# Takatsuka-Mark/Photogrammetry

Measured on AMD Instinct MI355X. Metric: descriptor pairs matched/sec, higher is better.
Workload: dtype u8 / bits (descriptor bits expanded to fp4 +-1 for the MFMA distance: exact integers in f32 accumulators; integer keys); f32 grey; 1 GPU; BASELINE configs[2] (SURVEY 8d config 3) x 1: 64-frame 1920x1080 RGBA64 sequence(s), dewarp(shipped coeffs)+gray+FAST(T=0.1)+NMS(r=16; SURVEY 8d writes r = 20 for this config: both leave more than 4096 survivors per frame, the lists are cut to the same length either way)+BRIEF-256 per frame, all 2016 ordered image pairs per sequence through the greedy Hamming match, <=4096 keypoints per frame (fir; frames=64, image_pairs=2016, frames_per_gpu=64, image_pairs_per_gpu=2016, parallelism=frames f mod 1, image pairs p mod 1; 2 all-gathers per step (elided at N = 1), jobs_in_flight=2, rehearsal_on_one_gpu_with_gloo=False

## Files before the change

### photogrammetry_amd/csrc/k_image.hip

```cpp
#include "pgx_internal.h"

namespace {

__device__ __forceinline__ float gray_of(uint2 px)
{
    float r = (float)(px.x & 0xFFFFu), g = (float)(px.x >> 16), b = (float)(px.y & 0xFFFFu);
    float s = __fadd_rn(__fadd_rn(r, b), g);
    return __fdiv_rn(s, 196605.0f);
}

constexpr int FB = 4;

__device__ __forceinline__ uint2 widen8(uint32_t v)
{
    return make_uint2(__builtin_amdgcn_perm(v, v, 0x01010000u), __builtin_amdgcn_perm(v, v, 0x03030202u));
}

template <bool SRC8> struct SrcPix { using type = uint2; };
template <> struct SrcPix<true> { using type = uint32_t; };
template <bool SRC8> __device__ __forceinline__ uint2 load_px(const typename SrcPix<SRC8>::type *p);
template <> __device__ __forceinline__ uint2 load_px<false>(const uint2 *p) { return *p; }
template <> __device__ __forceinline__ uint2 load_px<true>(const uint32_t *p) { return widen8(*p); }

template <bool HAS_MAP, bool WRITE_RGBA, bool SRC8>
__global__ __launch_bounds__(256) void k_dewarp_gray(const typename SrcPix<SRC8>::type *__restrict__ rgba,
                                                     const int2 *__restrict__ map, int W, int H, int F,
                                                     float *__restrict__ gray, uint2 *__restrict__ dewarped, int *status)
{
    using Px = typename SrcPix<SRC8>::type;
    const size_t npix = (size_t)W * H;
    const int f0 = blockIdx.y * FB;
    const int nf = F - f0 < FB ? F - f0 : FB;
    const size_t ngroups = (npix + 3) / 4;
    const bool vec = (npix & 3) == 0 || F == 1;
    bool oob = false;
    for (size_t grp = (size_t)blockIdx.x * blockDim.x + threadIdx.x; grp < ngroups;
         grp += (size_t)gridDim.x * blockDim.x) {
        const size_t i0 = grp * 4;
        if (vec && i0 + 3 < npix) {
            size_t so[4];
            bool ok[4];
            if (HAS_MAP) {
                const int4 m01 = *reinterpret_cast<const int4 *>(map + i0);
                const int4 m23 = *reinterpret_cast<const int4 *>(map + i0 + 2);
                const int us[4] = {m01.x, m01.z, m23.x, m23.z};
                const int vs[4] = {m01.y, m01.w, m23.y, m23.w};
#pragma unroll
                for (int k = 0; k < 4; k++) {
                    const unsigned su = (unsigned)us[k] & 0xFFFFu, sv = (unsigned)vs[k] & 0xFFFFu;
                    ok[k] = su < (unsigned)W && sv < (unsigned)H;
                    oob |= !ok[k];
                    so[k] = ok[k] ? (size_t)sv * W + su : 0;
                }
            }
            uint2 px[FB][4];
#pragma unroll
            for (int fb = 0; fb < FB; fb++) {
                if (fb >= nf) break;
                const Px *src = rgba + (size_t)(f0 + fb) * npix;
                if (HAS_MAP) {
#pragma unroll
                    for (int k = 0; k < 4; k++) px[fb][k] = load_px<SRC8>(src + so[k]);
                } else if constexpr (SRC8) {
                    const uint4 a = *reinterpret_cast<const uint4 *>(src + i0);
                    px[fb][0] = widen8(a.x); px[fb][1] = widen8(a.y); px[fb][2] = widen8(a.z); px[fb][3] = widen8(a.w);
                } else {
                    const uint4 a = *reinterpret_cast<const uint4 *>(src + i0);
                    const uint4 b = *reinterpret_cast<const uint4 *>(src + i0 + 2);
                    px[fb][0] = make_uint2(a.x, a.y); px[fb][1] = make_uint2(a.z, a.w);
                    px[fb][2] = make_uint2(b.x, b.y); px[fb][3] = make_uint2(b.z, b.w);
                }
            }
#pragma unroll
            for (int fb = 0; fb < FB; fb++) {
                if (fb >= nf) break;
                if (HAS_MAP) {
#pragma unroll
                    for (int k = 0; k < 4; k++) if (!ok[k]) px[fb][k] = make_uint2(0, 0);
                }
                if (gray) {
                    const float4 g4 = make_float4(gray_of(px[fb][0]), gray_of(px[fb][1]), gray_of(px[fb][2]), gray_of(px[fb][3]));
                    *reinterpret_cast<float4 *>(gray + (size_t)(f0 + fb) * npix + i0) = g4;
                }
                if (WRITE_RGBA) {
                    uint2 *dout = dewarped + (size_t)(f0 + fb) * npix;
                    *reinterpret_cast<uint4 *>(dout + i0) = make_uint4(px[fb][0].x, px[fb][0].y, px[fb][1].x, px[fb][1].y);
                    *reinterpret_cast<uint4 *>(dout + i0 + 2) = make_uint4(px[fb][2].x, px[fb][2].y, px[fb][3].x, px[fb][3].y);
                }
            }
        } else {
            for (size_t i = i0; i < npix && i < i0 + 4; i++) {
                size_t o = i;
                bool okk = true;
                if (HAS_MAP) {
                    const int2 m = map[i];
                    const unsigned su = (unsigned)m.x & 0xFFFFu, sv = (unsigned)m.y & 0xFFFFu;
                    okk = su < (unsigned)W && sv < (unsigned)H;
                    oob |= !okk;
                    o = okk ? (size_t)sv * W + su : 0;
                }
                for (int fb = 0; fb < nf; fb++) {
                    const uint2 p = okk ? load_px<SRC8>(rgba + (size_t)(f0 + fb) * npix + o) : make_uint2(0, 0);
                    if (gray) gray[(size_t)(f0 + fb) * npix + i] = gray_of(p);
                    if (WRITE_RGBA) dewarped[(size_t)(f0 + fb) * npix + i] = p;
                }
            }
        }
    }
    if (HAS_MAP && oob) atomicOr(status, (int)PGX_ST_OOB_SOURCE);
}

__device__ __forceinline__ int32_t trunc_to_int_dev(double v)
{
    if (!(v > -2147483649.0 && v < 2147483648.0)) return INT32_MIN;
    return (int32_t)v;
}

__device__ __forceinline__ double cbrt_signed_dev(double n)
{
    const double sgn = (double)((n > 0) - (n < 0));
    return pow(fabs(n), 1.0 / 3.0) * sgn;
}

__global__ __launch_bounds__(256) void k_dewarp_map(int W, int H, double k0, double k1, double k2, double k3, double k4,
                                                    int2 *__restrict__ map, int *status)
{
    const size_t i = (size_t)blockIdx.x * 256 + threadIdx.x;
    if (i >= (size_t)W * H) return;
    const int v = (int)(i / W), u = (int)(i - (size_t)v * W);
    const double x0 = W / 2.0, y0 = H / 2.0;
    const int x = trunc_to_int_dev(u - x0), y = trunc_to_int_dev(v - y0);
    const int rd2 = x * x + y * y;
    const double rd = sqrt((double)rd2);
    const double den = rd * k4 - k1;
    const double a2 = (rd * k3 - k0) / den, a1 = (rd * k2 - 1) / den, a0 = rd / den;
    const double Q = (3 * a1 - a2 * a2) / 9.0;
    const double R = (9.0 * a2 * a1 - 27 * a0 - 2 * a2 * a2 * a2) / 54.0;
    const double Q3 = Q * Q * Q;
    const double D = Q3 + R * R;
    const double shift = -a2 / 3.0;
    const double nan = __longlong_as_double(0x7FF8000000000000ll);
    double r0 = nan, r1 = nan, r2 = nan;
    if (D >= 0) {
        const double sqrtD = pow(D, 0.5);
        const double S = cbrt_signed_dev(R + sqrtD), T = cbrt_signed_dev(R - sqrtD);
        r0 = shift + (S + T);
        if (D == 0) r1 = shift - S;
    } else {
        const double pi = 3.1415926535897932384626433832795;
        const double theta = acos(R / sqrt(-Q3));
        const double m = 2.0 * sqrt(-Q);
        r0 = m * cos(theta / 3.0) + shift;
        r1 = m * cos((theta + 2.0 * pi) / 3.0) + shift;
        r2 = m * cos((theta - 2.0 * pi) / 3.0) + shift;
    }
    double kept[3];
    int n = 0;
    if (!isnan(r0)) kept[n++] = r0;
    if (!isnan(r1)) kept[n++] = r1;
    if (!isnan(r2)) kept[n++] = r2;
    if (n == 0) { atomicOr(status, (int)PGX_ST_INTERNAL); map[i] = make_int2(INT32_MIN, INT32_MIN); return; }
    if (n >= 2 && kept[0] > kept[1]) { const double t = kept[0]; kept[0] = kept[1]; kept[1] = t; }
    if (n == 3) {
        if (kept[1] > kept[2]) { const double t = kept[1]; kept[1] = kept[2]; kept[2] = t; }
        if (kept[0] > kept[1]) { const double t = kept[0]; kept[0] = kept[1]; kept[1] = t; }
    }
    const double root = n == 3 ? kept[1] : kept[0];
    const double theta = atan2((double)y, (double)x);
    map[i] = make_int2(trunc_to_int_dev(root * cos(theta) + x0), trunc_to_int_dev(root * sin(theta) + y0));
}

}

void pgx_launch_dewarp_gray(hipStream_t s, const void *rgba, int src8, const int32_t *map_uv, int F, int W, int H,
                            float *gray, uint16_t *dewarped, int *status)
{
    if (F <= 0 || W <= 0 || H <= 0) return;
    const size_t ngroups = ((size_t)W * H + 3) / 4;
    unsigned gx = (unsigned)((ngroups + 255) / 256);
    const unsigned ny = (unsigned)((F + FB - 1) / FB);
    const unsigned cap = 512u / ny > 32u ? 512u / ny : 32u;
    if (gx > cap) gx = cap;
    dim3 grid(gx, (unsigned)((F + FB - 1) / FB)), block(256);
    const int2 *map = reinterpret_cast<const int2 *>(map_uv);
    uint2 *dw = reinterpret_cast<uint2 *>(dewarped);
#define PGX_DG(M, WR, S8) hipLaunchKernelGGL((k_dewarp_gray<M, WR, S8>), grid, block, 0, s, \
                                             reinterpret_cast<const SrcPix<S8>::type *>(rgba), map, W, H, F, gray, dw, status)
    if (src8) {
        if (map) { if (dw) PGX_DG(true, true, true); else PGX_DG(true, false, true); }
        else { if (dw) PGX_DG(false, true, true); else PGX_DG(false, false, true); }
    } else {
        if (map) { if (dw) PGX_DG(true, true, false); else PGX_DG(true, false, false); }
        else { if (dw) PGX_DG(false, true, false); else PGX_DG(false, false, false); }
    }
#undef PGX_DG
}

void pgx_launch_dewarp_map(hipStream_t s, int W, int H, const double *k, int32_t *map_uv, int *status)
{
    const size_t npix = (size_t)W * H;
    hipLaunchKernelGGL(k_dewarp_map, dim3((unsigned)((npix + 255) / 256)), dim3(256), 0, s, W, H, k[0], k[1], k[2], k[3], k[4],
                       reinterpret_cast<int2 *>(map_uv), status);
}
```

### photogrammetry_amd/csrc/k_nms.hip

```cpp
#include "pgx_internal.h"
#include <cstdlib>

namespace {

constexpr int NT = 1024;
constexpr int WIDE_ROUNDS = 8;
constexpr uint32_t SORT_LDS_MAX = 16384;
constexpr uint32_t MT_SORT_LDS = 8192;

struct NmsLayout {
    int gw, gh, cs, ncell;
    int R;
    int champ;
    int cgw;
    int mask;
    size_t off_cellstart, off_cellfill, off_cellund, off_counters, off_rec, off_listA, off_listB, off_accflag, off_sortkeys,
        off_champ, off_alive, off_planes, off_disk, total;
};

__host__ __device__ inline int nms_champ_cs(int radius, int n_cap, bool planes)
{
    if (!planes || radius < 10 || radius > 192 || n_cap > (1 << 24)) return 0;
    return radius >= 90 ? 64 : (radius >= 44 ? 32 : (radius >= 22 ? 16 : 8));
}
// ... 749 lines not shown
        for (int t = q; t < ND * ND * 64; t += gridDim.x * 256) {
            const int o = t >> 6, pos = t & 63, ux = pos & 7, uy = pos >> 3;
            const int dx = o % ND - RR, dy = o / ND - RR;
            unsigned long long m = 0;
            for (int i = 0; i < 8; i++) {
                const int ddy = dy * 8 + i - uy, rem = r2 - ddy * ddy;
                if (rem < 0) continue;
                int hw = (int)sqrtf((float)rem);
                while ((hw + 1) * (hw + 1) <= rem) hw++;
                while (hw * hw > rem) hw--;
                int lo = ux - dx * 8 - hw, hi = ux - dx * 8 + hw;
                lo = lo < 0 ? 0 : lo;
                hi = hi > 7 ? 7 : hi;
                if (lo <= hi) m |= (unsigned long long)(((1u << (hi + 1)) - 1u) & ~((1u << lo) - 1u)) << (8 * i);
            }
            disk[t] = m;
        }
    }
    if (q >= npc) return;
    const MaskPtrs M = mask_ptrs(ws_all + (size_t)f * ws_stride, L);
    if (q < 16) M.counters[q] = 0;
    const int py = q / L.cgw, px = q - py * L.cgw;
    const int cx = px - RR, cy = py - RR;
    if (cx < 0 || cx >= L.gw || cy < 0 || cy >= L.gh) {
        M.alive[q] = 0ull;
        M.ent[q] = 0u;
        return;
    }
    const int x0 = cx * 8, tx = x0 >> 6, bo = x0 & 63;
    const int y0 = cy * 8, y1 = (y0 + 8 < H) ? y0 + 8 : H;
    const size_t nseg = (size_t)H * ntx;
    const unsigned long long *seg = seg_all + (size_t)f * nseg * 4;
    const bool over = n_raw_all[f] > n_cap;
    unsigned long long A0 = 0, A1 = 0, A2 = 0;
    ulonglong2 rp8[8];
    unsigned long long rb8[8];
#pragma unroll
    for (int i = 0; i < 8; i++) {
        const bool ok = y0 + i < y1;
        const size_t si = (size_t)(ok ? y0 + i : y0) * ntx + tx;
        rp8[i] = *reinterpret_cast<const ulonglong2 *>(seg + si * 4);
        rb8[i] = seg[si * 4 + 2];
        if (!ok) { rp8[i] = make_ulonglong2(0ull, 0ull); rb8[i] = 0ull; }
    }
#pragma unroll
    for (int i = 0; i < 8; i++) {
        const unsigned long long any = rp8[i].x | rp8[i].y | rb8[i];
        uint32_t keep = (uint32_t)(any >> bo) & 0xFFu;
        if (over && keep) {
            const uint32_t base = segoff_all[(size_t)f * nseg + (size_t)(y0 + i) * ntx + tx] + (uint32_t)__popcll(any & ((1ull << bo) - 1ull));
            const uint32_t room = base < (uint32_t)n_cap ? (uint32_t)n_cap - base : 0u;
            while ((uint32_t)__popc(keep) > room) keep &= ~(1u << (31 - __builtin_clz(keep)));
        }
        A0 |= ((rp8[i].x >> bo) & (unsigned long long)keep) << (8 * i);
        A1 |= ((rp8[i].y >> bo) & (unsigned long long)keep) << (8 * i);
        A2 |= ((rb8[i] >> bo) & (unsigned long long)keep) << (8 * i);
    }
    const unsigned long long a = A0 | A1 | A2;
    M.alive[q] = a;
    M.pl0[q] = A0; M.pl1[q] = A1; M.pl2[q] = A2;
    M.ent[q] = mask_champ(a, A0, A1, A2, cx, cy);
}

struct MaskOut { uint32_t *raw_xy; int32_t *raw_score; const unsigned long long *seg; const uint32_t *segoff; int ntx; };

__device__ __forceinline__ uint32_t ent_load(const uint32_t *p) { return __hip_atomic_load(p, __ATOMIC_RELAXED, __HIP_MEMORY_SCOPE_AGENT); }
__device__ __forceinline__ void ent_store(uint32_t *p, uint32_t v) { __hip_atomic_store(p, v, __ATOMIC_RELAXED, __HIP_MEMORY_SCOPE_AGENT); }


__device__ __forceinline__ bool mask_own(const MaskPtrs &M, int pc, int cx, int cy, bool incell, uint32_t &me, unsigned long long a,
                                         unsigned long long q0, unsigned long long q1, unsigned long long q2)
{
    if (!incell) return false;
    if (me & MK_FLAG) {
        ent_store(M.ent + pc, 0u);
        __hip_atomic_store(M.alive + pc, 0ull, __ATOMIC_RELAXED, __HIP_MEMORY_SCOPE_AGENT);
        return false;
    }
    if (a == 0ull) {
        if (me) ent_store(M.ent + pc, 0u);
        return false;
    }
    const uint32_t pos = 0x0FFFFFFFu - (me & 0x0FFFFFFFu);
    const int b = (int)((((pos >> 14) & 7u) << 3) | (pos & 7u));
    if (me == 0u || !((a >> b) & 1ull)) {
        me = mask_champ(a, q0, q1, q2, cx, cy);
        ent_store(M.ent + pc, me);
    }
    return true;
// ... 724 lines not shown
```

### photogrammetry_amd/csrc/pgx_api.hip

```cpp
#include "pgx_trackgraph.h"
#include "pgx_brief_plan.h"

#include <atomic>
#include <cmath>
#include <cstdarg>
#include <cstdio>
#include <new>
#include <cstring>
#include <cstdlib>

#define PGX_VERSION_STR "pgx 0.1 (gfx950)"

static thread_local std::string tl_err;
static thread_local const pgx_ctx *tl_err_ctx = nullptr;
static thread_local unsigned long long tl_err_id = 0;
static std::atomic<unsigned long long> g_ctx_ids{0};

void pgx_note_error(pgx_ctx *c, const std::string &msg)
{
    tl_err = msg;
    tl_err_ctx = c;
    tl_err_id = c ? c->id : 0;
    if (c) {
        std::lock_guard<std::mutex> g(c->err_mu);
// ... 164 lines not shown
        pgx_launch_fast(c->stream, gray, F, W, H, c->threshold, c->ws_seg.as<unsigned long long>(),
                        c->ws_segoff.as<uint32_t>(), d_nraw, c->ws_rawxy.as<uint32_t>(),
                        c->ws_rawscore.as<int32_t>(), raw_cap, c->d_status,
                        !pgx_nms_fills_raw_lists(W, H, c->radius, raw_cap));
    }
    {
        ProfScope ps(c, "nms");
        pgx_launch_nms(c->stream, c->ws_rawxy.as<uint32_t>(), c->ws_rawscore.as<int32_t>(), d_nraw, F, raw_cap, W, H,
                       c->radius, c->ws_nms.p, nms_stride, c->ws_order.as<uint32_t>(), c->ws_nkept.as<int32_t>(),
                       kp_eff, c->d_status, c->ws_seg.as<unsigned long long>(), c->ws_segoff.as<uint32_t>(), kp_soft);
    }
    {
        ProfScope ps(c, "brief");
        const PgxSteer st = steer_of(c, d_bins);
        pgx_launch_brief(c->stream, gray, F, W, H, c->ws_rawxy.as<uint32_t>(), c->ws_rawscore.as<int32_t>(), raw_cap,
                         c->ws_order.as<uint32_t>(), c->ws_nkept.as<int32_t>(), kp_eff, c->d_pairs.as<int32_t>(), c->d_plan.as<int32_t>(), c->P,
                         d_kp, d_desc, d_counts, out_stride, c->steer_on ? &st : nullptr);
    }
}

int enqueue_detect_bins(pgx_ctx *c, const uint16_t *d_rgba, int F, int W, int H, pgx_keypoint *d_kp, uint32_t *d_desc,
                        int32_t *d_counts, int32_t *d_nraw, int cap, int32_t *d_bins, int32_t *d_origin = nullptr,
                        int32_t *d_stats = nullptr)
{
    const int rcp = pgx_prepare_detect(c, F, W, H, cap);
    if (rcp != PGX_OK) return rcp;
    if (F <= 0) return PGX_OK;
    const bool kp_soft = c->kp_cap <= cap;
    const int kp_eff = kp_soft ? c->kp_cap : cap;

    float *gray = c->ws_gray.as<float>();
    {
        ProfScope ps(c, "dewarp_gray");
        pgx_launch_dewarp_gray(c->stream, d_rgba, c->src8, c->map_set ? c->d_map.as<int32_t>() : nullptr, F, W, H, gray,
                               nullptr, c->d_status);
    }
    if (c->pyr_levels <= 1) {
        enqueue_from_gray(c, gray, F, W, H, kp_eff, kp_soft, d_kp, d_desc, d_counts, d_nraw, cap, d_bins);
    } else {
        const PyrPlan pl = pyr_plan(c, W, H);
        int32_t *lvl_counts = c->ws_pyr_cnt.as<int32_t>(), *lvl_nraw = lvl_counts + (size_t)8 * F;
        const size_t lvl_slots = (size_t)F * kp_eff;
        int32_t *tmp_bins = d_bins ? c->ws_pyr_bins.as<int32_t>() : nullptr;
        enqueue_from_gray(c, gray, F, W, H, kp_eff, kp_soft, d_kp, d_desc, lvl_counts, lvl_nraw, cap, d_bins);
        const float *src = gray;
        for (int l = 1; l < pl.n_run; l++) {
            float *dst = (l & 1) ? c->ws_pyr_a.as<float>() : c->ws_pyr_b.as<float>();
            {
                ProfScope ps(c, "pyramid");
                pgx_launch_pyr_down(c->stream, src, F, pl.dims[l - 1][0], pl.dims[l - 1][1], dst, pl.dims[l][0], pl.dims[l][1],
                                    c->pyr_step);
            }
            enqueue_from_gray(c, dst, F, pl.dims[l][0], pl.dims[l][1], kp_eff, kp_soft,
                              c->ws_pyr_kp.as<pgx_keypoint>() + (l - 1) * lvl_slots,
                              c->ws_pyr_desc.as<uint32_t>() + (l - 1) * lvl_slots * c->words, lvl_counts + (size_t)l * F,
                              lvl_nraw + (size_t)l * F, kp_eff, tmp_bins ? tmp_bins + (l - 1) * lvl_slots : nullptr);
            src = dst;
        }
        {
            ProfScope ps(c, "pyramid_append");
            pgx_launch_pyr_append(c->stream, c->ws_pyr_kp.as<pgx_keypoint>(), c->ws_pyr_desc.as<uint32_t>(), tmp_bins, lvl_counts,
                                  lvl_nraw, F, kp_eff, c->words, pl.n_levels, pl.n_run, W, H, pl.scale, d_kp, d_desc, d_bins,
                                  d_counts, d_nraw, d_origin, d_stats, cap, c->d_status);
        }
    }
    HIPCHK(c, hipEventRecord(c->ev_stage[PGX_STAGE_DETECT], c->stream));
    HIPCHK(c, hipGetLastError());
// ... 114 lines not shown
    if (strncmp(prop.gcnArchName, "gfx950", 6) != 0) {
        fprintf(stderr, "pgx: device %d is %s; this library is built for gfx950 only\n", device, prop.gcnArchName);
        return PGX_E_HIP;
    }
    pgx_ctx *c = new (std::nothrow) pgx_ctx();
    if (!c) return PGX_E_HIP;
    c->device = device;
    c->id = ++g_ctx_ids;
    if (hipStreamCreateWithFlags(&c->own_stream, hipStreamNonBlocking) != hipSuccess ||
        hipEventCreateWithFlags(&c->ev_stage[0], hipEventDisableTiming) != hipSuccess ||
        hipEventCreateWithFlags(&c->ev_stage[1], hipEventDisableTiming) != hipSuccess ||
        hipEventCreateWithFlags(&c->ev_stage[2], hipEventDisableTiming) != hipSuccess ||
        hipEventCreateWithFlags(&c->ev_stage[3], hipEventDisableTiming) != hipSuccess ||
        hipMalloc(reinterpret_cast<void **>(&c->d_status), 256) != hipSuccess ||
        hipHostMalloc(reinterpret_cast<void **>(&c->h_status), 64, hipHostMallocDefault) != hipSuccess ||
        hipMemset(c->d_status, 0, 256) != hipSuccess) {
        pgx_ctx_destroy(c);
        return PGX_E_HIP;
    }
    c->stream = c->own_stream;
    *out = c;
    return PGX_OK;
}

void pgx_ctx_destroy(pgx_ctx *c)
{
    if (!c) return;
    (void)hipSetDevice(c->device);
    if (c->stream) (void)hipStreamSynchronize(c->stream);
    if (c->comm) (void)pgx_comm_destroy(c);
    for (auto &kv : c->prof)
        for (auto &ev : kv.second.pending) { (void)hipEventDestroy(ev.first); (void)hipEventDestroy(ev.second); }
    for (hipEvent_t ev : c->ev_pool) (void)hipEventDestroy(ev);
    DevBuf *bufs[] = {&c->d_pairs, &c->d_plan, &c->d_steer_pairs, &c->d_steer_plans, &c->d_steer_dirs, &c->d_map, &c->ws_gray, &c->ws_seg, &c->ws_segoff, &c->ws_nraw, &c->ws_rawxy,
                      &c->ws_rawscore, &c->ws_nms, &c->ws_order, &c->ws_nkept, &c->st_a, &c->st_b, &c->st_c,
                      &c->st_d, &c->st_e, &c->st_f, &c->ws_pose, &c->ws_tracks, &c->ws_tracks_split, &c->ws_agree, &c->ws_matchn[0], &c->ws_matchn[1], &c->ws_matchn[2], &c->ws_knn, &c->ws_guided, &c->ws_tri, &c->ws_ba, &c->ws_reg, &c->ws_ver, &c->ws_init,
                      &c->ws_pyr_a, &c->ws_pyr_b, &c->ws_pyr_kp, &c->ws_pyr_desc, &c->ws_pyr_bins, &c->ws_pyr_cnt};
    for (DevBuf *b : bufs) b->release();
    c->pin_in.release();
    c->pin_out.release();
    if (c->d_status) (void)hipFree(c->d_status);
    if (c->h_status) (void)hipHostFree(c->h_status);
    for (int k = 0; k < 3; k++) {
        if (c->mstream[k]) (void)hipStreamDestroy(c->mstream[k]);
        if (c->ev_wide[k]) (void)hipEventDestroy(c->ev_wide[k]);
        if (c->ev_rows[k]) (void)hipEventDestroy(c->ev_rows[k]);
        if (c->ev_fin[k]) (void)hipEventDestroy(c->ev_fin[k]);
        if (c->ev_join[k]) (void)hipEventDestroy(c->ev_join[k]);
    }
    if (c->ev_in) (void)hipEventDestroy(c->ev_in);
    for (int k = 0; k < 4; k++) if (c->ev_stage[k]) (void)hipEventDestroy(c->ev_stage[k]);
    if (c->own_stream) (void)hipStreamDestroy(c->own_stream);
    delete c;
}

const char *pgx_last_error(pgx_ctx *c)
{
    if (!c) return "null context";
    if (tl_err_ctx == c && tl_err_id == c->id) return tl_err.c_str();
    static thread_local std::string copy;
    {
        std::lock_guard<std::mutex> g(c->err_mu);
        copy = c->err;
    }
    return copy.c_str();
}

int pgx_set_stream(pgx_ctx *c, void *hip_stream)
{
    if (!c) return PGX_E_BADARG;
    Lock l(c);
    c->cfg_epoch++;
    HIPCHK(c, hipStreamSynchronize(c->stream));
    c->stream = hip_stream ? reinterpret_cast<hipStream_t>(hip_stream) : c->own_stream;
    return PGX_OK;
}

int pgx_check_status(pgx_ctx *c)
{
    if (!c) return PGX_E_BADARG;
    Lock l(c);
    return sync_status(c);
}

int pgx_set_dewarp_map(pgx_ctx *c, const int32_t *uv, int W, int H)
{
    if (!c) return PGX_E_BADARG;
    Lock l(c);
    c->cfg_epoch++;
    if (!uv) { c->map_set = false; c->mapW = c->mapH = 0; return PGX_OK; }
    if (dims_ok(c, W, H, "map dimensions must fit ushort") != PGX_OK) return PGX_E_BADARG;
    const size_t bytes = (size_t)W * H * 8;
    HIPCHK(c, hipStreamSynchronize(c->stream));
    HIPCHK(c, c->d_map.ensure(bytes + 32));
    HIPCHK(c, hipMemcpy(c->d_map.p, uv, bytes, hipMemcpyHostToDevice));
    c->mapW = W; c->mapH = H; c->map_set = true;
    return PGX_OK;
}

int pgx_set_dewarp_coeffs(pgx_ctx *c, int W, int H, const double *coeffs, int ncoeffs)
{
    if (!c || !coeffs) return c ? fail(c, PGX_E_BADARG, "null pointer") : PGX_E_BADARG;
    Lock l(c);
    c->cfg_epoch++;
    if (ncoeffs != 5) return fail(c, PGX_E_BADARG, "You must pass exactly 5 distortion coefficients (ArgumentException)");
    if (dims_ok(c, W, H, "map dimensions must fit ushort") != PGX_OK) return PGX_E_BADARG;
    const size_t bytes = (size_t)W * H * 8;
    HIPCHK(c, hipStreamSynchronize(c->stream));
    HIPCHK(c, c->d_map.ensure(bytes + 32));
    pgx_launch_dewarp_map(c->stream, W, H, coeffs, c->d_map.as<int32_t>(), c->d_status);
    HIPCHK(c, hipGetLastError());
    c->mapW = W; c->mapH = H; c->map_set = true;
    return sync_status(c);
}

int pgx_get_dewarp_map(pgx_ctx *c, int32_t *uv_out, int W, int H)
{
    if (!c || !uv_out) return c ? fail(c, PGX_E_BADARG, "null pointer") : PGX_E_BADARG;
    Lock l(c);
    if (!c->map_set) return fail(c, PGX_E_NOT_CONFIGURED, "no dewarp map is set");
    if (W != c->mapW || H != c->mapH) return fail(c, PGX_E_DIM_MISMATCH, "map is %dx%d, asked for %dx%d", c->mapW, c->mapH, W, H);
    HIPCHK(c, hipStreamSynchronize(c->stream));
    HIPCHK(c, hipMemcpy(uv_out, c->d_map.p, (size_t)W * H * 8, hipMemcpyDeviceToHost));
    return PGX_OK;
}

int pgx_set_brief_pairs(pgx_ctx *c, const int32_t *pairs, int P)
{
    if (!c) return PGX_E_BADARG;
    Lock l(c);
    c->cfg_epoch++;
    if (!pairs || P <= 0 || P > 4064) return fail(c, PGX_E_BADARG, "P must be in [1, 4064]");
    HIPCHK(c, hipStreamSynchronize(c->stream));
    HIPCHK(c, c->d_pairs.ensure((size_t)P * 16));
    HIPCHK(c, hipMemcpy(c->d_pairs.p, pairs, (size_t)P * 16, hipMemcpyHostToDevice));
    if (P == PGX_PLAN_PAIRS) {
        int32_t plan[PGX_PLAN_WORDS];
        pgx_build_brief_plan(pairs, plan);
        HIPCHK(c, c->d_plan.ensure(sizeof plan));
        HIPCHK(c, hipMemcpy(c->d_plan.p, plan, sizeof plan, hipMemcpyHostToDevice));
    }
    c->P = P; c->words = (P + 31) / 32; c->pairs_set = true;
    c->steer_on = false;
// ... 82 lines not shown

int pgx_set_source_format(pgx_ctx *c, int format)
{
    if (!c) return PGX_E_BADARG;
    Lock l(c);
    c->cfg_epoch++;
    if (format != PGX_SRC_RGBA64 && format != PGX_SRC_RGBA8) return fail(c, PGX_E_BADARG, "unknown source format %d", format);
    c->src8 = format == PGX_SRC_RGBA8;
    return PGX_OK;
}

int pgx_set_capacity(pgx_ctx *c, int max_raw, int max_kp)
{
    if (!c) return PGX_E_BADARG;
    Lock l(c);
    c->cfg_epoch++;
    if (max_raw <= 0 || max_kp <= 0 || max_kp > (1 << PGX_IDX_BITS)) return fail(c, PGX_E_BADARG, "bad capacity");
    c->raw_cap = max_raw; c->kp_cap = max_kp;
    return PGX_OK;
}


int pgx_dewarp(pgx_ctx *c, const uint16_t *rgba, int W, int H, uint16_t *out)
{
    if (!c || !rgba || !out) return c ? fail(c, PGX_E_BADARG, "null pointer") : PGX_E_BADARG;
    Lock l(c);
    if (!c->map_set) return fail(c, PGX_E_NOT_CONFIGURED, "pgx_set_dewarp_map not called");
    if (W != c->mapW || H != c->mapH)
        return fail(c, PGX_E_DIM_MISMATCH, "image %dx%d vs dewarp map %dx%d (ArgumentException)", W, H, c->mapW, c->mapH);
    const size_t bytes = (size_t)W * H * 8, in_bytes = (size_t)W * H * (c->src8 ? 4 : 8);
    HIPCHK(c, c->st_a.ensure(bytes + 32));
    HIPCHK(c, c->st_b.ensure(bytes + 32));
    HIPCHK(c, hipMemcpyAsync(c->st_a.p, rgba, in_bytes, hipMemcpyHostToDevice, c->stream));
    pgx_launch_dewarp_gray(c->stream, c->st_a.p, c->src8, c->d_map.as<int32_t>(), 1, W, H, nullptr,
                           c->st_b.as<uint16_t>(), c->d_status);
    HIPCHK(c, hipMemcpyAsync(out, c->st_b.p, bytes, hipMemcpyDeviceToHost, c->stream));
    return sync_status(c);
}

int pgx_gray(pgx_ctx *c, const uint16_t *rgba, int W, int H, float *out)
{
    if (!c || !rgba || !out) return c ? fail(c, PGX_E_BADARG, "null pointer") : PGX_E_BADARG;
    Lock l(c);
    if (dims_ok(c, W, H) != PGX_OK) return PGX_E_BADARG;
    const size_t npix = (size_t)W * H;
    HIPCHK(c, c->st_a.ensure(npix * 8 + 32));
    HIPCHK(c, c->st_b.ensure(npix * 4 + 32));
    HIPCHK(c, hipMemcpyAsync(c->st_a.p, rgba, npix * (c->src8 ? 4 : 8), hipMemcpyHostToDevice, c->stream));
    pgx_launch_dewarp_gray(c->stream, c->st_a.p, c->src8, nullptr, 1, W, H, c->st_b.as<float>(), nullptr,
                           c->d_status);
    HIPCHK(c, hipMemcpyAsync(out, c->st_b.p, npix * 4, hipMemcpyDeviceToHost, c->stream));
    return sync_status(c);
}

int pgx_fast(pgx_ctx *c, const float *gray, int W, int H, pgx_keypoint *out, int capacity, int *n_out)
{
    if (!c || !gray || !n_out || (capacity > 0 && !out) || capacity < 0)
        return c ? fail(c, PGX_E_BADARG, "null pointer") : PGX_E_BADARG;
    Lock l(c);
    if (!c->params_set) return fail(c, PGX_E_NOT_CONFIGURED, "pgx_set_detect_params not called");
    if (dims_ok(c, W, H) != PGX_OK) return PGX_E_BADARG;
    const size_t npix = (size_t)W * H, nseg = pgx_fast_seg_count(W, H);
    const int cap = capacity > 0 ? capacity : 1;
    HIPCHK(c, c->st_a.ensure(npix * 4 + 32));
    HIPCHK(c, c->ws_seg.ensure(nseg * 32));
    HIPCHK(c, c->ws_segoff.ensure(nseg * 4));
    HIPCHK(c, c->ws_nraw.ensure(64));
// ... 1087 lines not shown
```

### photogrammetry_amd/csrc/pgx_internal.h

```cpp
#pragma once

#include <hip/hip_runtime.h>
#include <stdint.h>

#include <map>
#include <mutex>
#include <string>
#include <type_traits>
#include <utility>
#include <vector>

#include "../../include/pgx.h"

#define PGX_ST_OOB_SOURCE 1u
#define PGX_ST_RAW_CAP    2u
#define PGX_ST_KP_CAP     4u
#define PGX_ST_EMPTY_SET  8u
#define PGX_ST_INTERNAL   16u
#define PGX_ST_BADARG     32u
#define PGX_ST_DUP_FRAME  64u
#define PGX_ST_TRI_CAP    128u
#define PGX_ST_TRI_NODE   256u
#define PGX_ST_TRI_DUP    512u
#define PGX_ST_BA_CAP     1024u
// ... 46 lines not shown
    }
    void release() { if (p) (void)hipHostFree(p); p = nullptr; cap = 0; }
    template <class T> T *as() const { return reinterpret_cast<T *>(p); }
};

struct ProfEntry {
    std::vector<std::pair<hipEvent_t, hipEvent_t>> pending;
    int launches = 0;
    double total_ms = 0.0;
};

struct pgx_ctx {
    int device = 0;
    hipStream_t own_stream = nullptr;
    hipStream_t stream = nullptr;
    std::mutex mu;
    std::string err;
    std::mutex err_mu;

    float threshold = 0.f;
    int radius = 0;
    bool params_set = false;
    int P = 0, words = 0;
    bool pairs_set = false;
    DevBuf d_pairs;
    DevBuf d_plan;
    bool steer_on = false;
    int steer_B = 0, steer_R = 0;
    DevBuf d_steer_pairs, d_steer_plans, d_steer_dirs;
    int pyr_levels = 1, pyr_step = 0;
    int mapW = 0, mapH = 0;
    bool map_set = false;
    DevBuf d_map;
    int raw_cap = 1 << 17;
    int kp_cap = 1 << PGX_IDX_BITS;
    int match_chunk = 2048;
    int src8 = 0;

    int *d_status = nullptr;
    int *h_status = nullptr;

    DevBuf ws_gray, ws_seg, ws_segoff, ws_nraw, ws_rawxy, ws_rawscore, ws_nms, ws_order, ws_nkept;
    DevBuf ws_pyr_a, ws_pyr_b, ws_pyr_kp, ws_pyr_desc, ws_pyr_bins, ws_pyr_cnt;
    DevBuf st_a, st_b, st_c, st_d, st_e, st_f;
    PinBuf pin_in, pin_out;
    DevBuf ws_matchn[3];
    DevBuf ws_pose, ws_tracks;
    DevBuf ws_tracks_split;
    DevBuf ws_knn;
    DevBuf ws_guided;
    DevBuf ws_tri;
    DevBuf ws_ba;
    DevBuf ws_reg;
    DevBuf ws_ver;
    DevBuf ws_init;
    hipStream_t mstream[3] = {nullptr, nullptr, nullptr};
    hipEvent_t ev_in = nullptr, ev_wide[3] = {nullptr, nullptr, nullptr}, ev_rows[3] = {nullptr, nullptr, nullptr},
               ev_fin[3] = {nullptr, nullptr, nullptr}, ev_join[3] = {nullptr, nullptr, nullptr};
    hipEvent_t ev_stage[4] = {nullptr, nullptr, nullptr, nullptr};
    hipEvent_t match_gate = nullptr;

    void *comm = nullptr;
    int comm_rank = 0, comm_world = 1;
    std::string comm_agreed;
    unsigned cfg_epoch = 0;
    unsigned long long id = 0;
// ... 25 lines not shown
    }
}
#endif

void pgx_note_error(pgx_ctx *c, const std::string &msg);

struct ProfScope {
    pgx_ctx *c;
    ProfEntry *e = nullptr;
    hipEvent_t a = nullptr, b = nullptr;
    hipStream_t st;
    bool attach;
    ProfScope(pgx_ctx *ctx, const char *name, hipStream_t s = nullptr, bool attach_to_kernel = false)
        : c(ctx), st(s ? s : ctx->stream), attach(attach_to_kernel)
    {
        if (!name || !c->prof_on || (!c->prof_only.empty() && c->prof_only != name)) return;
        e = &c->prof[name];
        auto take = [&](hipEvent_t &ev) {
            if (!c->ev_pool.empty()) { ev = c->ev_pool.back(); c->ev_pool.pop_back(); return true; }
            return hipEventCreate(&ev) == hipSuccess;
        };
        if (!take(a) || !take(b)) { e = nullptr; a = b = nullptr; return; }
        if (!attach) (void)hipEventRecord(a, st);
    }
    ~ProfScope()
    {
        if (!e) return;
        if (!attach) (void)hipEventRecord(b, st);
        e->pending.emplace_back(a, b);
    }
};


void pgx_launch_dewarp_gray(hipStream_t s, const void *rgba, int src8, const int32_t *map_uv, int F, int W, int H,
                            float *gray, uint16_t *dewarped, int *status);
void pgx_launch_dewarp_map(hipStream_t s, int W, int H, const double *k , int32_t *map_uv, int *status);

size_t pgx_fast_seg_count(int W, int H);
void pgx_launch_fast(hipStream_t s, const float *gray, int F, int W, int H, float T,
                     unsigned long long *seg , uint32_t *segoff ,
                     int32_t *n_raw , uint32_t *raw_xy ,
                     int32_t *raw_score , int raw_cap, int *status,
                     bool compact = true );

size_t pgx_nms_ws_bytes(int W, int H, int radius, int n_cap, bool planes);
bool pgx_nms_fills_raw_lists(int W, int H, int radius, int n_cap);
void pgx_launch_nms(hipStream_t s, uint32_t *raw_xy, int32_t *raw_score, const int32_t *n_raw,
                    int F, int n_cap, int W, int H, int radius, void *ws, size_t ws_stride,
                    uint32_t *order , int32_t *n_kept , int kp_cap, int *status,
                    const unsigned long long *seg = nullptr ,
                    const uint32_t *segoff = nullptr,
                    bool kp_soft = false );
hipError_t pgx_launch_nms_sync(hipStream_t s, const uint32_t *raw_xy, const int32_t *raw_score, const int32_t *n_raw,
                               int n_cap, int W, int H, int radius, void *ws, size_t ws_stride, uint32_t *order,
                               int32_t *n_kept, int kp_cap, int *status);

struct PgxSteer {
    const int32_t *pairs_rot;
    const int32_t *plans;
    const int32_t *dirs;
    int B, R;
    int32_t *bins_out;
};

void pgx_launch_brief(hipStream_t s, const float *gray, int F, int W, int H,
                      const uint32_t *raw_xy, const int32_t *raw_score, int raw_cap,
                      const uint32_t *order, const int32_t *n_kept, int kp_cap ,
                      const int32_t *pairs, const int32_t *plan , int P,
                      pgx_keypoint *kp_out, uint32_t *desc_out, int32_t *counts_out, int out_stride ,
// ... 102 lines not shown
```

Baseline: 5004 billion descriptor pairs/s.

## Pack dewarp map to 32-bit, pipeline frame loads, and slim NMS segment reads

The dewarp map is packed once into 16+16-bit coordinates, which halves the bytes each map read costs. The dewarp-gray kernel moves to 32-bit indexing, loads raw pixels two frames at a time with a non-unrolled outer loop, and allows more workgroups. The NMS seeding path now reads single bytes per row for the common not-over-cap case and only falls back to the popcount trimming when over cap. This adds a pack kernel and a second map buffer, and 32-bit indexing assumes frame sizes fit in 32 bits.

New measurement: 5031 billion descriptor pairs/s (median of 6 runs). About the same (+0.5%).

```diff
diff --git a/photogrammetry_amd/csrc/k_image.hip b/photogrammetry_amd/csrc/k_image.hip
--- a/photogrammetry_amd/csrc/k_image.hip
+++ b/photogrammetry_amd/csrc/k_image.hip
@@ -10,6 +10,8 @@
 }
 
 constexpr int FB = 4;
+constexpr unsigned DG_WGS = 1024;
+constexpr int FP = 2;
 
 __device__ __forceinline__ uint2 widen8(uint32_t v)
 {
@@ -21,83 +23,104 @@
 template <bool SRC8> __device__ __forceinline__ uint2 load_px(const typename SrcPix<SRC8>::type *p);
 template <> __device__ __forceinline__ uint2 load_px<false>(const uint2 *p) { return *p; }
 template <> __device__ __forceinline__ uint2 load_px<true>(const uint32_t *p) { return widen8(*p); }
+__device__ __forceinline__ uint2 wide_px(uint2 v) { return v; }
+__device__ __forceinline__ uint2 wide_px(uint32_t v) { return widen8(v); }
+
+__device__ __forceinline__ void after(float &g, uint2 &p) { asm volatile("" : "+v"(g), "+v"(p.x)); }
+__device__ __forceinline__ void after(float &g, uint32_t &p) { asm volatile("" : "+v"(g), "+v"(p)); }
+
+__device__ __forceinline__ uint32_t src_pixel(uint32_t m, int W, int H, bool &ok)
+{
+    const uint32_t su = m & 0xFFFFu, sv = m >> 16;
+    ok = su < (uint32_t)W && sv < (uint32_t)H;
+    return ok ? sv * (uint32_t)W + su : 0u;
+}
 
 template <bool HAS_MAP, bool WRITE_RGBA, bool SRC8>
 __global__ __launch_bounds__(256) void k_dewarp_gray(const typename SrcPix<SRC8>::type *__restrict__ rgba,
-                                                     const int2 *__restrict__ map, int W, int H, int F,
+                                                     const uint32_t *__restrict__ map, int W, int H, int F,
                                                      float *__restrict__ gray, uint2 *__restrict__ dewarped, int *status)
 {
     using Px = typename SrcPix<SRC8>::type;
-    const size_t npix = (size_t)W * H;
+    const uint32_t npix = (uint32_t)W * (uint32_t)H;
     const int f0 = blockIdx.y * FB;
     const int nf = F - f0 < FB ? F - f0 : FB;
-    const size_t ngroups = (npix + 3) / 4;
-    const bool vec = (npix & 3) == 0 || F == 1;
+    const uint32_t ngroups = (npix + 3u) / 4u;
+    const bool vec = (npix & 3u) == 0 || F == 1;
     bool oob = false;
-    for (size_t grp = (size_t)blockIdx.x * blockDim.x + threadIdx.x; grp < ngroups;
-         grp += (size_t)gridDim.x * blockDim.x) {
-        const size_t i0 = grp * 4;
-        if (vec && i0 + 3 < npix) {
-            size_t so[4];
-            bool ok[4];
+    for (uint32_t grp = blockIdx.x * 256u + threadIdx.x; grp < ngroups; grp += gridDim.x * 256u) {
+        const uint32_t i0 = grp * 4u;
+        if (vec && i0 + 3u < npix) {
+            uint32_t so[4];
+            uint32_t bad = 0;
             if (HAS_MAP) {
-                const int4 m01 = *reinterpret_cast<const int4 *>(map + i0);
-                const int4 m23 = *reinterpret_cast<const int4 *>(map + i0 + 2);
-                const int us[4] = {m01.x, m01.z, m23.x, m23.z};
-                const int vs[4] = {m01.y, m01.w, m23.y, m23.w};
+                const uint4 m = *reinterpret_cast<const uint4 *>(map + i0);
+                const uint32_t ms[4] = {m.x, m.y, m.z, m.w};
 #pragma unroll
                 for (int k = 0; k < 4; k++) {
-                    const unsigned su = (unsigned)us[k] & 0xFFFFu, sv = (unsigned)vs[k] & 0xFFFFu;
-                    ok[k] = su < (unsigned)W && sv < (unsigned)H;
-                    oob |= !ok[k];
-                    so[k] = ok[k] ? (size_t)sv * W + su : 0;
-                }
+                    bool ok;
+                    so[k] = src_pixel(ms[k], W, H, ok);
+                    bad |= ok ? 0u : 1u << k;
+                }
+                oob |= bad != 0u;
             }
-            uint2 px[FB][4];
-#pragma unroll
-            for (int fb = 0; fb < FB; fb++) {
-                if (fb >= nf) break;
-                const Px *src = rgba + (size_t)(f0 + fb) * npix;
-                if (HAS_MAP) {
-#pragma unroll
-                    for (int k = 0; k < 4; k++) px[fb][k] = load_px<SRC8>(src + so[k]);
-                } else if constexpr (SRC8) {
-                    const uint4 a = *reinterpret_cast<const uint4 *>(src + i0);
-                    px[fb][0] = widen8(a.x); px[fb][1] = widen8(a.y); px[fb][2] = widen8(a.z); px[fb][3] = widen8(a.w);
-                } else {
-                    const uint4 a = *reinterpret_cast<const uint4 *>(src + i0);
-                    const uint4 b = *reinterpret_cast<const uint4 *>(src + i0 + 2);
-                    px[fb][0] = make_uint2(a.x, a.y); px[fb][1] = make_uint2(a.z, a.w);
-                    px[fb][2] = make_uint2(b.x, b.y); px[fb][3] = make_uint2(b.z, b.w);
-                }
-            }
-#pragma unroll
-            for (int fb = 0; fb < FB; fb++) {
-                if (fb >= nf) break;
-                if (HAS_MAP) {
-#pragma unroll
-                    for (int k = 0; k < 4; k++) if (!ok[k]) px[fb][k] = make_uint2(0, 0);
-                }
-                if (gray) {
-                    const float4 g4 = make_float4(gray_of(px[fb][0]), gray_of(px[fb][1]), gray_of(px[fb][2]), gray_of(px[fb][3]));
-                    *reinterpret_cast<float4 *>(gray + (size_t)(f0 + fb) * npix + i0) = g4;
-                }
-                if (WRITE_RGBA) {
-                    uint2 *dout = dewarped + (size_t)(f0 + fb) * npix;
-                    *reinterpret_cast<uint4 *>(dout + i0) = make_uint4(px[fb][0].x, px[fb][0].y, px[fb][1].x, px[fb][1].y);
-                    *reinterpret_cast<uint4 *>(dout + i0 + 2) = make_uint4(px[fb][2].x, px[fb][2].y, px[fb][3].x, px[fb][3].y);
+            constexpr int fp = WRITE_RGBA ? 1 : FP;
+#pragma unroll 1
+            for (int fb = 0; fb < nf; fb += fp) {
+                Px raw[fp][4];
+#pragma unroll
+                for (int j = 0; j < fp; j++) {
+                    if (fb + j >= nf) break;
+                    const Px *src = rgba + (size_t)(f0 + fb + j) * npix;
+                    if (HAS_MAP) {
+#pragma unroll
+                        for (int k = 0; k < 4; k++) {
+                            uint32_t o = so[k];
+                            asm volatile("" : "+v"(o));
+                            raw[j][k] = src[o];
+                        }
+                    } else if constexpr (SRC8) {
+                        const uint4 a = *reinterpret_cast<const uint4 *>(src + i0);
+                        raw[j][0] = a.x; raw[j][1] = a.y; raw[j][2] = a.z; raw[j][3] = a.w;
+                    } else {
+                        const uint4 a = *reinterpret_cast<const uint4 *>(src + i0);
+                        const uint4 b = *reinterpret_cast<const uint4 *>(src + i0 + 2);
+                        raw[j][0] = make_uint2(a.x, a.y); raw[j][1] = make_uint2(a.z, a.w);
+                        raw[j][2] = make_uint2(b.x, b.y); raw[j][3] = make_uint2(b.z, b.w);
+                    }
+                }
+#pragma unroll
+                for (int j = 0; j < fp; j++) {
+                    if (fb + j >= nf) break;
+                    const size_t fo = (size_t)(f0 + fb + j) * npix + i0;
+                    if (HAS_MAP) {
+#pragma unroll
+                        for (int k = 0; k < 4; k++) if (bad >> k & 1u) raw[j][k] = Px{};
+                    }
+                    if (WRITE_RGBA) {
+                        const uint2 p0 = wide_px(raw[j][0]), p1 = wide_px(raw[j][1]);
+                        *reinterpret_cast<uint4 *>(dewarped + fo) = make_uint4(p0.x, p0.y, p1.x, p1.y);
+                        const uint2 p2 = wide_px(raw[j][2]), p3 = wide_px(raw[j][3]);
+                        *reinterpret_cast<uint4 *>(dewarped + fo + 2) = make_uint4(p2.x, p2.y, p3.x, p3.y);
+                    }
+                    if (gray) {
+                        float g[4];
+#pragma unroll
+                        for (int k = 0; k < 4; k++) {
+                            g[k] = gray_of(wide_px(raw[j][k]));
+                            if (WRITE_RGBA && k < 3) after(g[k], raw[j][k + 1]);
+                        }
+                        *reinterpret_cast<float4 *>(gray + fo) = make_float4(g[0], g[1], g[2], g[3]);
+                    }
                 }
             }
         } else {
-            for (size_t i = i0; i < npix && i < i0 + 4; i++) {
-                size_t o = i;
+            for (uint32_t i = i0; i < npix && i < i0 + 4u; i++) {
+                uint32_t o = i;
                 bool okk = true;
                 if (HAS_MAP) {
-                    const int2 m = map[i];
-                    const unsigned su = (unsigned)m.x & 0xFFFFu, sv = (unsigned)m.y & 0xFFFFu;
-                    okk = su < (unsigned)W && sv < (unsigned)H;
+                    o = src_pixel(map[i], W, H, okk);
                     oob |= !okk;
-                    o = okk ? (size_t)sv * W + su : 0;
                 }
                 for (int fb = 0; fb < nf; fb++) {
                     const uint2 p = okk ? load_px<SRC8>(rgba + (size_t)(f0 + fb) * npix + o) : make_uint2(0, 0);
@@ -108,6 +131,14 @@
         }
     }
     if (HAS_MAP && oob) atomicOr(status, (int)PGX_ST_OOB_SOURCE);
+}
+
+__global__ __launch_bounds__(256) void k_dewarp_pack(const int2 *__restrict__ map, uint32_t *__restrict__ packed, uint32_t npix)
+{
+    const uint32_t i = blockIdx.x * 256u + threadIdx.x;
+    if (i >= npix) return;
+    const int2 m = map[i];
+    packed[i] = ((uint32_t)m.x & 0xFFFFu) | ((uint32_t)m.y & 0xFFFFu) << 16;
 }
 
 __device__ __forceinline__ int32_t trunc_to_int_dev(double v)
@@ -172,17 +203,16 @@
 
 }
 
-void pgx_launch_dewarp_gray(hipStream_t s, const void *rgba, int src8, const int32_t *map_uv, int F, int W, int H,
+void pgx_launch_dewarp_gray(hipStream_t s, const void *rgba, int src8, const uint32_t *map, int F, int W, int H,
                             float *gray, uint16_t *dewarped, int *status)
 {
     if (F <= 0 || W <= 0 || H <= 0) return;
     const size_t ngroups = ((size_t)W * H + 3) / 4;
     unsigned gx = (unsigned)((ngroups + 255) / 256);
     const unsigned ny = (unsigned)((F + FB - 1) / FB);
-    const unsigned cap = 512u / ny > 32u ? 512u / ny : 32u;
+    const unsigned cap = DG_WGS / ny > 32u ? DG_WGS / ny : 32u;
     if (gx > cap) gx = cap;
     dim3 grid(gx, (unsigned)((F + FB - 1) / FB)), block(256);
-    const int2 *map = reinterpret_cast<const int2 *>(map_uv);
     uint2 *dw = reinterpret_cast<uint2 *>(dewarped);
 #define PGX_DG(M, WR, S8) hipLaunchKernelGGL((k_dewarp_gray<M, WR, S8>), grid, block, 0, s, \
                                              reinterpret_cast<const SrcPix<S8>::type *>(rgba), map, W, H, F, gray, dw, status)
@@ -202,3 +232,9 @@
     hipLaunchKernelGGL(k_dewarp_map, dim3((unsigned)((npix + 255) / 256)), dim3(256), 0, s, W, H, k[0], k[1], k[2], k[3], k[4],
                        reinterpret_cast<int2 *>(map_uv), status);
 }
+
+void pgx_launch_dewarp_pack(hipStream_t s, int W, int H, const int32_t *map_uv, uint32_t *packed)
+{
+    const uint32_t npix = (uint32_t)W * (uint32_t)H;
+    hipLaunchKernelGGL(k_dewarp_pack, dim3((npix + 255u) / 256u), dim3(256), 0, s, reinterpret_cast<const int2 *>(map_uv), packed, npix);
+}
diff --git a/photogrammetry_amd/csrc/k_nms.hip b/photogrammetry_amd/csrc/k_nms.hip
--- a/photogrammetry_amd/csrc/k_nms.hip
+++ b/photogrammetry_amd/csrc/k_nms.hip
@@ -805,29 +805,53 @@
     const size_t nseg = (size_t)H * ntx;
     const unsigned long long *seg = seg_all + (size_t)f * nseg * 4;
     const bool over = n_raw_all[f] > n_cap;
+    const unsigned char *segb = reinterpret_cast<const unsigned char *>(seg);
+    const uint32_t cell_off = (uint32_t)tx * 32u + (uint32_t)(bo >> 3), row_bytes = (uint32_t)ntx * 32u;
+    const uint32_t off0 = (uint32_t)y0 * row_bytes + cell_off;
+    const int nr = y1 - y0;
     unsigned long long A0 = 0, A1 = 0, A2 = 0;
-    ulonglong2 rp8[8];
-    unsigned long long rb8[8];
-#pragma unroll
-    for (int i = 0; i < 8; i++) {
-        const bool ok = y0 + i < y1;
-        const size_t si = (size_t)(ok ? y0 + i : y0) * ntx + tx;
-        rp8[i] = *reinterpret_cast<const ulonglong2 *>(seg + si * 4);
-        rb8[i] = seg[si * 4 + 2];
-        if (!ok) { rp8[i] = make_ulonglong2(0ull, 0ull); rb8[i] = 0ull; }
-    }
-#pragma unroll
-    for (int i = 0; i < 8; i++) {
-        const unsigned long long any = rp8[i].x | rp8[i].y | rb8[i];
-        uint32_t keep = (uint32_t)(any >> bo) & 0xFFu;
-        if (over && keep) {
-            const uint32_t base = segoff_all[(size_t)f * nseg + (size_t)(y0 + i) * ntx + tx] + (uint32_t)__popcll(any & ((1ull << bo) - 1ull));
-            const uint32_t room = base < (uint32_t)n_cap ? (uint32_t)n_cap - base : 0u;
-            while ((uint32_t)__popc(keep) > room) keep &= ~(1u << (31 - __builtin_clz(keep)));
-        }
-        A0 |= ((rp8[i].x >> bo) & (unsigned long long)keep) << (8 * i);
-        A1 |= ((rp8[i].y >> bo) & (unsigned long long)keep) << (8 * i);
-        A2 |= ((rb8[i] >> bo) & (unsigned long long)keep) << (8 * i);
+    if (!over) {
+        uint32_t l0 = 0, l1 = 0, l2 = 0, h0 = 0, h1 = 0, h2 = 0;
+#pragma unroll 1
+        for (int half = 0; half < 2; half++) {
+            uint32_t b[4][3];
+#pragma unroll
+            for (int i = 0; i < 4; i++) {
+                const int r = half * 4 + i;
+                const uint32_t o = off0 + __umul24((uint32_t)(r < nr ? r : nr - 1), row_bytes);
+#pragma unroll
+                for (int p = 0; p < 3; p++) b[i][p] = segb[o + 8u * p];
+            }
+            const uint32_t w0 = b[0][0] | b[1][0] << 8 | b[2][0] << 16 | b[3][0] << 24;
+            const uint32_t w1 = b[0][1] | b[1][1] << 8 | b[2][1] << 16 | b[3][1] << 24;
+            const uint32_t w2 = b[0][2] | b[1][2] << 8 | b[2][2] << 16 | b[3][2] << 24;
+            if (half == 0) { l0 = w0; l1 = w1; l2 = w2; } else { h0 = w0; h1 = w1; h2 = w2; }
+        }
+        const unsigned long long in = nr == 8 ? ~0ull : (1ull << (8 * nr)) - 1ull;
+        A0 = ((unsigned long long)h0 << 32 | l0) & in;
+        A1 = ((unsigned long long)h1 << 32 | l1) & in;
+        A2 = ((unsigned long long)h2 << 32 | l2) & in;
+    } else {
+#pragma unroll 1
+        for (int y = y0; y < y1; y++) {
+            const uint32_t off = off0 + __umul24((uint32_t)(y - y0), row_bytes);
+            const uint32_t b0 = segb[off], b1 = segb[off + 8u], b2 = segb[off + 16u];
+            uint32_t keep = b0 | b1 | b2;
+            if (keep) {
+                const uint32_t wo = off - (uint32_t)(bo >> 3);
+                const uint2 *sw = reinterpret_cast<const uint2 *>(segb + wo);
+                const uint2 p0 = sw[0], p1 = sw[1], p2 = sw[2];
+                const uint32_t lo = p0.x | p1.x | p2.x, hi = p0.y | p1.y | p2.y;
+                const uint32_t below = bo < 32 ? __popc(lo & ((1u << bo) - 1u)) : __popc(lo) + __popc(hi & ((1u << (bo - 32)) - 1u));
+                const uint32_t base = *reinterpret_cast<const uint32_t *>(reinterpret_cast<const unsigned char *>(segoff_all + (size_t)f * nseg) + (wo >> 3)) + below;
+                const uint32_t room = base < (uint32_t)n_cap ? (uint32_t)n_cap - base : 0u;
+                while ((uint32_t)__popc(keep) > room) keep &= ~(1u << (31 - __builtin_clz(keep)));
+            }
+            const int sh = 8 * (y - y0);
+            A0 |= (unsigned long long)(b0 & keep) << sh;
+            A1 |= (unsigned long long)(b1 & keep) << sh;
+            A2 |= (unsigned long long)(b2 & keep) << sh;
+        }
     }
     const unsigned long long a = A0 | A1 | A2;
     M.alive[q] = a;
diff --git a/photogrammetry_amd/csrc/pgx_api.hip b/photogrammetry_amd/csrc/pgx_api.hip
--- a/photogrammetry_amd/csrc/pgx_api.hip
+++ b/photogrammetry_amd/csrc/pgx_api.hip
@@ -220,7 +220,7 @@
     float *gray = c->ws_gray.as<float>();
     {
         ProfScope ps(c, "dewarp_gray");
-        pgx_launch_dewarp_gray(c->stream, d_rgba, c->src8, c->map_set ? c->d_map.as<int32_t>() : nullptr, F, W, H, gray,
+        pgx_launch_dewarp_gray(c->stream, d_rgba, c->src8, c->map_set ? c->d_map4.as<uint32_t>() : nullptr, F, W, H, gray,
                                nullptr, c->d_status);
     }
     if (c->pyr_levels <= 1) {
@@ -401,7 +401,7 @@
     for (auto &kv : c->prof)
         for (auto &ev : kv.second.pending) { (void)hipEventDestroy(ev.first); (void)hipEventDestroy(ev.second); }
     for (hipEvent_t ev : c->ev_pool) (void)hipEventDestroy(ev);
-    DevBuf *bufs[] = {&c->d_pairs, &c->d_plan, &c->d_steer_pairs, &c->d_steer_plans, &c->d_steer_dirs, &c->d_map, &c->ws_gray, &c->ws_seg, &c->ws_segoff, &c->ws_nraw, &c->ws_rawxy,
+    DevBuf *bufs[] = {&c->d_pairs, &c->d_plan, &c->d_steer_pairs, &c->d_steer_plans, &c->d_steer_dirs, &c->d_map, &c->d_map4, &c->ws_gray, &c->ws_seg, &c->ws_segoff, &c->ws_nraw, &c->ws_rawxy,
                       &c->ws_rawscore, &c->ws_nms, &c->ws_order, &c->ws_nkept, &c->st_a, &c->st_b, &c->st_c,
                       &c->st_d, &c->st_e, &c->st_f, &c->ws_pose, &c->ws_tracks, &c->ws_tracks_split, &c->ws_agree, &c->ws_matchn[0], &c->ws_matchn[1], &c->ws_matchn[2], &c->ws_knn, &c->ws_guided, &c->ws_tri, &c->ws_ba, &c->ws_reg, &c->ws_ver, &c->ws_init,
                       &c->ws_pyr_a, &c->ws_pyr_b, &c->ws_pyr_kp, &c->ws_pyr_desc, &c->ws_pyr_bins, &c->ws_pyr_cnt};
@@ -462,7 +462,11 @@
     const size_t bytes = (size_t)W * H * 8;
     HIPCHK(c, hipStreamSynchronize(c->stream));
     HIPCHK(c, c->d_map.ensure(bytes + 32));
+    HIPCHK(c, c->d_map4.ensure(bytes / 2 + 32));
     HIPCHK(c, hipMemcpy(c->d_map.p, uv, bytes, hipMemcpyHostToDevice));
+    pgx_launch_dewarp_pack(c->stream, W, H, c->d_map.as<int32_t>(), c->d_map4.as<uint32_t>());
+    HIPCHK(c, hipGetLastError());
+    HIPCHK(c, hipStreamSynchronize(c->stream));
     c->mapW = W; c->mapH = H; c->map_set = true;
     return PGX_OK;
 }
@@ -477,7 +481,9 @@
     const size_t bytes = (size_t)W * H * 8;
     HIPCHK(c, hipStreamSynchronize(c->stream));
     HIPCHK(c, c->d_map.ensure(bytes + 32));
+    HIPCHK(c, c->d_map4.ensure(bytes / 2 + 32));
     pgx_launch_dewarp_map(c->stream, W, H, coeffs, c->d_map.as<int32_t>(), c->d_status);
+    pgx_launch_dewarp_pack(c->stream, W, H, c->d_map.as<int32_t>(), c->d_map4.as<uint32_t>());
     HIPCHK(c, hipGetLastError());
     c->mapW = W; c->mapH = H; c->map_set = true;
     return sync_status(c);
@@ -626,7 +632,7 @@
     HIPCHK(c, c->st_a.ensure(bytes + 32));
     HIPCHK(c, c->st_b.ensure(bytes + 32));
     HIPCHK(c, hipMemcpyAsync(c->st_a.p, rgba, in_bytes, hipMemcpyHostToDevice, c->stream));
-    pgx_launch_dewarp_gray(c->stream, c->st_a.p, c->src8, c->d_map.as<int32_t>(), 1, W, H, nullptr,
+    pgx_launch_dewarp_gray(c->stream, c->st_a.p, c->src8, c->d_map4.as<uint32_t>(), 1, W, H, nullptr,
                            c->st_b.as<uint16_t>(), c->d_status);
     HIPCHK(c, hipMemcpyAsync(out, c->st_b.p, bytes, hipMemcpyDeviceToHost, c->stream));
     return sync_status(c);
diff --git a/photogrammetry_amd/csrc/pgx_internal.h b/photogrammetry_amd/csrc/pgx_internal.h
--- a/photogrammetry_amd/csrc/pgx_internal.h
+++ b/photogrammetry_amd/csrc/pgx_internal.h
@@ -102,6 +102,7 @@
     int mapW = 0, mapH = 0;
     bool map_set = false;
     DevBuf d_map;
+    DevBuf d_map4;
     int raw_cap = 1 << 17;
     int kp_cap = 1 << PGX_IDX_BITS;
     int match_chunk = 2048;
@@ -193,9 +194,10 @@
 };
 
 
-void pgx_launch_dewarp_gray(hipStream_t s, const void *rgba, int src8, const int32_t *map_uv, int F, int W, int H,
+void pgx_launch_dewarp_gray(hipStream_t s, const void *rgba, int src8, const uint32_t *map, int F, int W, int H,
                             float *gray, uint16_t *dewarped, int *status);
 void pgx_launch_dewarp_map(hipStream_t s, int W, int H, const double *k , int32_t *map_uv, int *status);
+void pgx_launch_dewarp_pack(hipStream_t s, int W, int H, const int32_t *map_uv, uint32_t *packed);
 
 size_t pgx_fast_seg_count(int W, int H);
 void pgx_launch_fast(hipStream_t s, const float *gray, int F, int W, int H, float T,
```
